# microsoft/Tokenizer

Measured on AMD Instinct MI355X. Metric: input MB/s encoded (cl100k_base), higher is better.
Workload: dtype u8

## Files before the change

tokenizer_amd/csrc/tkz_kernels.hip:

```cpp
#include "tkz_kernels.h"

#include <type_traits>

#include "tkz_bpe.h"
#include "tkz_classes.h"
#include "tkz_corpus.h"
#include "tkz_pretok.h"
#include "tkz_simt.h"

namespace tkz {

TKZ_KERNEL(256) void k_docmark(const int64_t* offs, int64_t n_items, int64_t total, uint64_t* bits, int32_t* counters) {
    const int64_t stride = simt::nblocks() * simt::nthreads();
    for (int64_t d = simt::bid() * simt::nthreads() + simt::tid(); d <= n_items; d += stride) {
        const int64_t pos = offs[d];
        bool ok = pos >= 0 && pos <= total;
        if (d == 0) ok = ok && pos == 0;
        if (d == n_items) ok = ok && pos == total;
        else ok = ok && pos <= offs[d + 1];
        if (!ok) { simt::atomic_or((unsigned*)&counters[0], (unsigned)kErrOffsets); continue; }
        const int64_t w = pos >> 6;
        if (d > 0) { const int64_t prev = offs[d - 1]; if (prev >= 0 && prev <= pos && (prev >> 6) == w) continue; }
        uint64_t m = 1ull << (pos & 63);
        int64_t cur = pos;
// ... 463 lines not shown
    const int w = (s >> 2) + i;
    const uint32_t x = simt::alignbit(s_bytes[w + 1], s_bytes[w], (uint32_t)(s & 3) * 8u);
    const int nb = len - 4 * i;
    return nb >= 4 ? x : (nb <= 0 ? 0u : (x & ((1u << (8 * nb)) - 1u)));
}

constexpr int kProbeLdsBytes = (kSub + kHalo) + 2 * (kSub + 2) + 2 * kMidMax + 4 * kMidMax + 4 * (kSub / 32);
constexpr int kProbeLdsQuads = (kProbeLdsBytes + 15) / 16;
struct ProbeLds { uint32_t* bytes; uint16_t* pstart; uint16_t* mid; uint32_t* midres; uint32_t* mark; const uint4* kmask; };
TKZ_DEV ProbeLds tkz_probe_lds(uint4* wave_quads, const uint4* kmask) {
    ProbeLds L;
    uint8_t* b = reinterpret_cast<uint8_t*>(wave_quads);
    L.bytes = reinterpret_cast<uint32_t*>(b); b += kSub + kHalo;
    L.midres = reinterpret_cast<uint32_t*>(b); b += 4 * kMidMax;
    L.mark = reinterpret_cast<uint32_t*>(b); b += 4 * (kSub / 32);
    L.pstart = reinterpret_cast<uint16_t*>(b); b += 2 * (kSub + 2);
    L.mid = reinterpret_cast<uint16_t*>(b);
    L.kmask = kmask;
    return L;
}
TKZ_DEV void tkz_probe_kmask_init(uint4* s_kmask) {
    if (simt::tid() <= TKZ_SHORT_KEY_MAX) {
        const int len = simt::tid();
        uint32_t m[3];
        for (int i = 0; i < 3; ++i) { const int nb = len - 4 * i; m[i] = nb >= 4 ? 0xFFFFFFFFu : (nb <= 0 ? 0u : ((1u << (8 * nb)) - 1u)); }
        uint4 v; v.x = m[0]; v.y = m[1]; v.z = m[2]; v.w = 0;
        s_kmask[len] = v;
    }
}
struct ProbeText { uint4 v0, v1; };
static_assert((kSub + kHalo) / 16 <= 128, "two 16-byte loads per lane cover the sub-tile and its halo");
TKZ_DEV void tkz_probe_request_text(const EncodeParams& P, int64_t sub, ProbeText* tx) {
    const int lane = simt::lane();
    const int64_t base = sub * kSub;
    uint4 v0, v1;
    v0.x = v0.y = v0.z = v0.w = 0; v1 = v0;
    const int64_t p0 = base + 16 * (int64_t)lane, p1 = base + 16 * (int64_t)(lane + 64);
    if (p0 + 16 <= P.total) v0 = tkz_load16_nt(P.bytes + p0);
    else {
        uint32_t w[4] = {0, 0, 0, 0};
        for (int j = 0; j < 16; ++j) if (p0 + j < P.total) w[j >> 2] |= (uint32_t)P.bytes[p0 + j] << (8 * (j & 3));
        v0.x = w[0]; v0.y = w[1]; v0.z = w[2]; v0.w = w[3];
    }
    if (lane + 64 < (kSub + kHalo) / 16) {
        if (p1 + 16 <= P.total) v1 = tkz_load16_nt(P.bytes + p1);
        else {
            uint32_t w[4] = {0, 0, 0, 0};
            for (int j = 0; j < 16; ++j) if (p1 + j < P.total) w[j >> 2] |= (uint32_t)P.bytes[p1 + j] << (8 * (j & 3));
            v1.x = w[0]; v1.y = w[1]; v1.z = w[2]; v1.w = w[3];
        }
    }
    tx->v0 = v0; tx->v1 = v1;
}
template <bool REPORT>
TKZ_DEV void tkz_probe_subtile(const TkzTables& T, const EncodeParams& P, int64_t sub, const ProbeLds& LD, ProbeText& tx, int64_t next) {
    const int lane = simt::lane();
    uint32_t* s_bytes = LD.bytes;
    uint16_t* s_pstart = LD.pstart;
    uint16_t* s_mid = LD.mid;
    uint32_t* s_midres = LD.midres;
    uint32_t* s_mark = LD.mark;
    const uint4* s_kmask = LD.kmask;
    const uint8_t* sb = reinterpret_cast<const uint8_t*>(s_bytes);
    const int64_t base = sub * kSub;
    const int nb = (int)(P.total - base < kSub ? P.total - base : kSub);
    const uint8_t* gbase = P.bytes + base;
    const bool prof = TKZ_DEV_FLAG(P, 16);
    long long t_0 = prof ? simt::clock() : 0, t_1 = 0, t_2 = 0, t_3 = 0;
    uint4 v0 = tx.v0, v1 = tx.v1;
    uint64_t myword = 0, mymark = 0;
    if (lane < kSub / 64) {
        const int64_t w = sub * (kSub / 64) + lane;
        if (w < P.nwords) { myword = P.startbits[w]; mymark = P.docbits[w]; }
    }
    const int64_t from = base + nb, w0 = from >> 6;
    uint64_t ahead = (w0 + lane < P.nwords) ? P.startbits[w0 + lane] : 0ull;
    const int64_t pb = P.pbase[sub];
    { uint4* s4 = reinterpret_cast<uint4*>(s_bytes); s4[lane] = v0; if (lane + 64 < (kSub + kHalo) / 16) s4[lane + 64] = v1; }
    if (next >= 0) tkz_probe_request_text(P, next, &tx);
    if (lane < kSub / 64) {
        const int lim = nb - lane * 64;
        if (lim <= 0) myword = 0; else if (lim < 64) myword &= tkz_lowmask(lim);
        s_mark[2 * lane] = (uint32_t)mymark; s_mark[2 * lane + 1] = (uint32_t)(mymark >> 32);
    }
    int64_t last_end;
    {
        int64_t found = -1;
        for (int64_t c = 0; found < 0; ++c) {
            const int64_t w = w0 + c * 64 + lane;
            uint64_t v = c == 0 ? ahead : (w < P.nwords ? P.startbits[w] : 0);
            if (w == w0) v &= ~tkz_lowmask((int)(from & 63));
            const uint64_t any = simt::ballot(v != 0);
            if (any) {
                const int src = tkz_ctz64(any);
                const uint32_t lo = simt::shflu((uint32_t)v, src), hi = simt::shflu((uint32_t)(v >> 32), src);
                found = ((w0 + c * 64 + src) << 6) + tkz_ctz64(((uint64_t)hi << 32) | lo);
            } else if (w0 + (c + 1) * 64 >= P.nwords) found = P.total;
        }
        last_end = found;
    }
    const int last_end_rel = (int)(last_end - base < 2 * kSub + 2 ? last_end - base : 2 * kSub + 2);
    const uint32_t wlo = simt::shflu((uint32_t)myword, lane >> 2), whi = simt::shflu((uint32_t)(myword >> 32), lane >> 2);
    const uint32_t bits16 = (uint32_t)(((((uint64_t)whi << 32) | wlo) >> (16 * (lane & 3))) & 0xFFFFull);
    int np;
    {
        int off = tkz_wave_scan<5>(tkz_popc32(bits16), &np);
        for (uint32_t b = bits16; b; b &= b - 1) s_pstart[off++] = (uint16_t)(16 * lane + tkz_ctz32(b));
        if (lane == 0) s_pstart[np] = (uint16_t)last_end_rel;
    }
    (void)simt::ballot(true);
    if (prof) t_1 = simt::clock();
    const char* tb0 = reinterpret_cast<const char*>(T.short_slots);
    const uint32_t mid_off = (uint32_t)(reinterpret_cast<const char*>(T.mid_slots) - tb0);
    int nmid = 0;
#pragma unroll 1
    for (int k0 = 0; k0 < np; k0 += 64) {
        const int k = k0 + lane;
        int len = 0;
        if (k < np) len = (int)s_pstart[k + 1] - (int)s_pstart[k];
        const uint64_t midm = simt::ballot(len > TKZ_SHORT_KEY_MAX && len <= kArenaPiece);
        if ((midm >> lane) & 1ull) s_mid[nmid + tkz_popc64(midm & tkz_lowmask(lane))] = (uint16_t)k;
        nmid += tkz_popc64(midm);
    }
    (void)simt::ballot(true);
#pragma unroll 1
    for (int m0 = 0; m0 < nmid; m0 += 64) {
        const bool valid = m0 + lane < nmid;
        int s = 0, len = 13;
        uint32_t kk[7] = {0, 0, 0, 0, 0, 0, 0}, oa = 0, ob = 0;
        if (valid) {
            const int k = s_mid[m0 + lane];
            s = s_pstart[k];
            len = (int)s_pstart[k + 1] - s;
        }
        const bool is_mid = valid && len <= TKZ_MID_KEY_MAX;
        if (is_mid) {
#pragma unroll
            for (int i = 0; i < 7; ++i) kk[i] = tkz_key_dword(s_bytes, s, len, i);
            uint32_t s1, s2;
            tkz_mid_slots(T, kk, (uint32_t)len, &s1, &s2);
            oa = mid_off + 32u * s1; ob = mid_off + 32u * s2;
        }
        const uint4 a0 = tkz_load16(tb0 + oa), a1 = tkz_load16(tb0 + oa + 16u), b0 = tkz_load16(tb0 + ob), b1 = tkz_load16(tb0 + ob + 16u);
        int32_t rank = TKZ_RANK_NONE;
        if (is_mid) rank = tkz_match_mid(kk, (uint32_t)len, a0, a1, b0, b1);
        else if (valid) {
            if (s + len <= kSub + kHalo) rank = tkz_lookup_long(T, [&](int i) -> uint32_t { return sb[s + i]; }, (uint32_t)len);
            else rank = tkz_lookup_long(T, [&](int i) -> uint32_t { return gbase[s + i]; }, (uint32_t)len);
        }
        if (valid) s_midres[m0 + lane] = (uint32_t)rank;
    }
    (void)simt::ballot(true);
    if (prof) t_2 = simt::clock();
    uint32_t* const ml = P.mlist + sub * (int64_t)P.mcap;
    uint4* const mq = P.mquad + sub * (int64_t)P.mcap;
    int ns = 0, nl = 0, midseen = 0;
    int promo_extra = 0;
    bool giant = false, coopl = false;
    constexpr int U = TKZ_PROBE_U;
#ifdef TKZ_DEVPROF
    long long pf_first = 0, pf_second = 0, pf_emit = 0, pf_t = 0;
    int pf_batches = 0, pf_valid = 0, pf_want2 = 0, pf_iters2 = 0;
#define TKZ_PROBE_MARK(acc) do { if (prof) { const long long pf_now = simt::clock(); acc += pf_now - pf_t; pf_t = pf_now; } } while (0)
    if (prof) pf_t = simt::clock();
#else
#define TKZ_PROBE_MARK(acc) do { } while (0)
#endif
#pragma unroll 1
    for (int k0 = 0; k0 < np; k0 += 64 * U) {
        int ps[U], plen[U];
        uint32_t hs[U], kw0[U], kw1[U], kw2[U];
        uint4 a0[U], a1[U];
#pragma unroll
        for (int u = 0; u < U; ++u) {
            const int k = k0 + 64 * u + lane;
            ps[u] = 0; plen[u] = 0;
            if (k < np) { ps[u] = s_pstart[k]; plen[u] = (int)s_pstart[k + 1] - ps[u]; }
            const int s = ps[u], w = s >> 2;
            const uint32_t sh = (uint32_t)(s & 3) * 8u;
            const uint32_t d0 = s_bytes[w], d1 = s_bytes[w + 1], d2 = s_bytes[w + 2], d3 = s_bytes[w + 3];
            const bool is_short = plen[u] >= 1 && plen[u] <= TKZ_SHORT_KEY_MAX;
            const uint4 km = s_kmask[is_short ? plen[u] : 0];
            kw0[u] = simt::alignbit(d1, d0, sh) & km.x; kw1[u] = simt::alignbit(d2, d1, sh) & km.y; kw2[u] = simt::alignbit(d3, d2, sh) & km.z;
            const uint32_t slot = tkz_short_slot_first(T, kw0[u], kw1[u], kw2[u], (uint32_t)plen[u], &hs[u]);
            const uint32_t oa = is_short ? 16u * slot : 0u;
            a0[u] = tkz_load16(tb0 + oa); a1[u] = tkz_load16(tb0 + oa + 16u);
        }
        int32_t rk[U];
        bool more = false;
#pragma unroll
        for (int u = 0; u < U; ++u) {
            const bool is_short = plen[u] >= 1 && plen[u] <= TKZ_SHORT_KEY_MAX;
            rk[u] = tkz_match_short2x(kw0[u], kw1[u], kw2[u], (uint32_t)plen[u], a0[u], a1[u]);
            more = more || (is_short && rk[u] == TKZ_RANK_NONE);
        }
        bool two_pass = simt::ballot(more) != 0;
        TKZ_PROBE_MARK(pf_first);
#ifdef TKZ_DEVPROF
        if (prof) {
            for (int u = 0; u < U; ++u) { const int nv = np - (k0 + 64 * u); if (nv > 0) { ++pf_batches; pf_valid += nv < 64 ? nv : 64; } }
            for (int u = 0; u < U; ++u) pf_want2 += tkz_popc64(simt::ballot(plen[u] >= 1 && plen[u] <= TKZ_SHORT_KEY_MAX && rk[u] == TKZ_RANK_NONE));
            pf_iters2 += two_pass ? 1 : 0;
            pf_t = simt::clock();
        }
#endif
        if (two_pass) {
#pragma unroll
            for (int u = 0; u < U; ++u) {
                const bool want = plen[u] >= 1 && plen[u] <= TKZ_SHORT_KEY_MAX && rk[u] == TKZ_RANK_NONE;
                if (want) {
                    const uint32_t ob = 16u * tkz_short_slot_second(T, hs[u]);
                    a0[u] = tkz_load16(tb0 + ob); a1[u] = tkz_load16(tb0 + ob + 16u);
                }
            }
#pragma unroll
            for (int u = 0; u < U; ++u) {
                const bool want = plen[u] >= 1 && plen[u] <= TKZ_SHORT_KEY_MAX && rk[u] == TKZ_RANK_NONE;
                if (want) rk[u] = tkz_match_short2x(kw0[u], kw1[u], kw2[u], (uint32_t)plen[u], a0[u], a1[u]);
            }
        }
        TKZ_PROBE_MARK(pf_second);
#pragma unroll
        for (int u = 0; u < U; ++u) {
            const int k = k0 + 64 * u + lane;
            const bool valid = k < np;
            const int s = ps[u], len = plen[u];
            const bool is_mid = len > TKZ_SHORT_KEY_MAX && len <= kArenaPiece;
            const uint64_t midm = simt::ballot(is_mid);
            int32_t rank = rk[u];
            if (is_mid) rank = (int32_t)s_midres[midseen + tkz_popc64(midm & tkz_lowmask(lane))];
            midseen += tkz_popc64(midm);
            const bool is_giant = len > kArenaPiece;
            const bool miss = valid && !is_giant && rank == TKZ_RANK_NONE;
            if (P.pextra) {
                const uint32_t ex = (valid && !is_giant && !miss && ((uint32_t)rank & kPromoFlag)) ? (((uint32_t)rank >> kPromoCntShift) & 3u) : 0u;
                promo_extra += (int)ex;
            }
            const bool miss_s = miss && len <= kShortMax, miss_l = miss && len > kShortMax;
            const uint64_t sm = simt::ballot(miss_s), lm = simt::ballot(miss_l);
            const int is_ = ns + tkz_popc64(sm & tkz_lowmask(lane)), il = nl + tkz_popc64(lm & tkz_lowmask(lane));
            ns += tkz_popc64(sm); nl += tkz_popc64(lm);
            const uint32_t ent = (uint32_t)s | ((uint32_t)(len - 1) << kMrLenShift);
            if (miss_s && is_ + nl < P.mcap) {
                ml[is_] = ent;
                uint4 kq; kq.x = kw0[u]; kq.y = kw1[u]; kq.z = kw2[u]; kq.w = 0;
                if (len > TKZ_SHORT_KEY_MAX) { kq.x = tkz_key_dword(s_bytes, s, len, 0); kq.y = tkz_key_dword(s_bytes, s, len, 1); kq.z = tkz_key_dword(s_bytes, s, len, 2); kq.w = tkz_key_dword(s_bytes, s, len, 3); }
                mq[is_] = kq;
            }
            if (miss_l && il + ns < P.mcap) ml[P.mcap - 1 - il] = ent;
            uint32_t rec = ((s_mark[s >> 5] >> (s & 31)) & 1u) ? kPrMark : 0u;
            if (REPORT) giant = giant || (miss_l && len > kSmallLanePiece);
            else coopl = coopl || (miss_l && len > P.lane_piece);
            if (is_giant) { rec |= kPrMiss | kPrGiant | (uint32_t)s; giant = giant || valid; }
            else if (miss) rec |= kPrMiss | (miss_l ? (kPrLong | (uint32_t)il) : (uint32_t)is_);
            else rec |= (uint32_t)rank;
            if (valid && pb + k < P.prank_cap) tkz_store_nt(&P.prank[pb + k], (int32_t)rec);
        }
        TKZ_PROBE_MARK(pf_emit);
    }
#undef TKZ_PROBE_MARK
#ifdef TKZ_DEVPROF
    if (prof && lane == 0) {
        simt::atomic_add64(&P.devprof[48], (unsigned long long)pf_first); simt::atomic_add64(&P.devprof[49], (unsigned long long)pf_second);
        simt::atomic_add64(&P.devprof[50], (unsigned long long)pf_emit); simt::atomic_add64(&P.devprof[51], (unsigned long long)pf_batches);
        simt::atomic_add64(&P.devprof[52], (unsigned long long)pf_valid); simt::atomic_add64(&P.devprof[53], (unsigned long long)pf_want2);
        simt::atomic_add64(&P.devprof[54], (unsigned long long)pf_iters2);
    }
#endif
    if (prof && lane == 0) {
        t_3 = simt::clock();
        simt::atomic_add64(&P.devprof[0], 1); simt::atomic_add64(&P.devprof[1], (unsigned long long)(t_3 - t_0));
        simt::atomic_add64(&P.devprof[2], (unsigned long long)(t_1 - t_0)); simt::atomic_add64(&P.devprof[3], (unsigned long long)(t_3 - t_2));
        simt::atomic_add64(&P.devprof[4], (unsigned long long)(t_2 - t_1)); simt::atomic_add64(&P.devprof[5], (unsigned long long)nmid);
        simt::atomic_add64(&P.devprof[6], (unsigned long long)np);
    }
    const uint32_t f = (nl ? 1u : 0u) | (simt::ballot(giant) ? 2u : 0u) | (simt::ballot(coopl) ? 4u : 0u);
    if (P.pextra) { int tot; (void)tkz_wave_scan_sum(promo_extra, &tot); promo_extra = tot; }
    if (lane == 0) {
        P.heavy_flag[sub] = (uint8_t)f;
        P.mcount[sub] = (uint32_t)ns | ((uint32_t)nl << 16);
        if (P.pextra) P.pextra[sub] = promo_extra;
        if (!REPORT && P.tc_atomic) P.tile_count[sub] = 0;
        if (REPORT && ns + nl > P.mcap) { simt::atomic_or((unsigned*)&P.counters[0], (unsigned)kErrMissCap); simt::atomic_max((unsigned*)&P.counters[1], (unsigned)(ns + nl)); }
        if (pb + np > P.prank_cap) simt::atomic_or((unsigned*)&P.counters[0], (unsigned)kErrCapacity);
    }
}
TKZ_KERNEL_OCC(256, TKZ_PROBE_OCC) void k_probe(TkzTables T, EncodeParams P) {
    TKZ_SHARED uint4 s_wave[kThreads / 64][kProbeLdsQuads];
    TKZ_SHARED uint4 s_kmask[TKZ_SHORT_KEY_MAX + 1];
    tkz_probe_kmask_init(s_kmask);
    simt::sync();
    const int64_t sub0 = (tkz_xcd_block(simt::bid(), simt::nblocks()) * (kThreads / 64) + simt::wave()) * kProbePer;
    if (sub0 >= P.nsub) return;
    const ProbeLds LD = tkz_probe_lds(s_wave[simt::wave()], s_kmask);
    ProbeText tx;
    tkz_probe_request_text(P, sub0, &tx);
#pragma unroll 1
    for (int it = 0; it < kProbePer && sub0 + it < P.nsub; ++it) {
        const int64_t nxt = (it + 1 < kProbePer && sub0 + it + 1 < P.nsub) ? sub0 + it + 1 : -1;
        tkz_probe_subtile<false>(T, P, sub0 + it, LD, tx, nxt);
        (void)simt::ballot(true);
    }
}

struct alignas(4) TkzDwords4 { uint32_t x, y, z, w; };
TKZ_DEV void tkz_load_piece16(const uint8_t* bytes, int64_t total, int64_t abs, uint32_t* pw) {
    const int64_t a0 = abs & ~(int64_t)3;
    const uint32_t sh = (uint32_t)(abs & 3) * 8u;
    uint32_t w[5];
    if (a0 + 20 <= total) {
        const TkzDwords4 v = *reinterpret_cast<const TkzDwords4*>(bytes + a0);
        w[0] = v.x; w[1] = v.y; w[2] = v.z; w[3] = v.w;
        w[4] = *reinterpret_cast<const uint32_t*>(bytes + a0 + 16);
    } else {
#pragma unroll
        for (int i = 0; i < 5; ++i) {
            const int64_t p = a0 + 4 * i;
            if (p + 4 <= total) w[i] = *reinterpret_cast<const uint32_t*>(bytes + p);
            else { w[i] = 0; for (int j = 0; j < 4; ++j) if (p + j < total) w[i] |= (uint32_t)bytes[p + j] << (8 * j); }
        }
    }
#pragma unroll
    for (int i = 0; i < 4; ++i) pw[i] = simt::alignbit(w[i + 1], w[i], sh);
}

TKZ_HD uint32_t tkz_result_entry(bool dense, int cnt, int off) { return kMrDone | (dense ? kMrDense : 0u) | ((uint32_t)(cnt - 1) << kMrCntShift) | (uint32_t)off; }
TKZ_HD uint32_t tkz_result_inline(int cnt) { return kMrDone | kMrInline | ((uint32_t)(cnt - 1) << kMrCntShift); }
TKZ_HD int tkz_result_cnt(uint32_t r) { return (int)((r >> kMrCntShift) & 1023u) + 1; }
TKZ_HD int tkz_result_off(uint32_t r) { return (int)(r & kMrOffMask); }

template <int N, class Pre>
TKZ_DEV int tkz_find_list(const Pre* pre, int g) {
    int q = 0;
#pragma unroll
    for (int step = N / 2; step >= 1; step >>= 1) if (pre[q + step] <= g) q += step;
    return q;
}

constexpr int kMsStride = TkzBpeGeom<16>::kStride, kMsIdStride = TkzBpeGeom<16>::kIdStride;
#ifndef TKZ_MS_SHORT_LEN
#define TKZ_MS_SHORT_LEN 8
#endif
#ifndef TKZ_MS_TWO_MIN
#define TKZ_MS_TWO_MIN 320
#endif
constexpr int kMsTwoListsMin = TKZ_MS_TWO_MIN;
constexpr int kMsShortLen = TKZ_MS_SHORT_LEN;
struct MsLds { uint4* pr; uint32_t* ids; uint16_t* rec; uint16_t* idx; int* extra; uint16_t* pre; const uint16_t* brank16; };
constexpr int kMsLdsBytes = kMsStride * 64 * 4 + kMsIdStride * 64 * 4 + 2 * (2 * 64 + 2 * 64) + 4 * kGroup + 2 * (kGroup + 1);
constexpr int kMsLdsQuads = (kMsLdsBytes + 15) / 16;
static_assert((kMsThreads / 64) * kMsLdsQuads * 16 + 512 <= 40960, "k_merge_short: four workgroups a CU (160 KB of LDS, allocated in units of 1,280 bytes)");
TKZ_DEV MsLds tkz_ms_lds(uint4* wave_quads, const uint16_t* brank16) {
    MsLds L;
    uint8_t* b = reinterpret_cast<uint8_t*>(wave_quads);
    L.pr = reinterpret_cast<uint4*>(b); b += kMsStride * 64 * 4;
    L.ids = reinterpret_cast<uint32_t*>(b); b += kMsIdStride * 64 * 4;
    L.extra = reinterpret_cast<int*>(b); b += 4 * kGroup;
    L.rec = reinterpret_cast<uint16_t*>(b); b += 2 * 2 * 64;
    L.idx = reinterpret_cast<uint16_t*>(b); b += 2 * 2 * 64;
    L.pre = reinterpret_cast<uint16_t*>(b);
    L.brank16 = brank16;
    return L;
}
TKZ_DEV void tkz_ms_brank_init(const TkzTables& T, uint16_t* s_brank16) {
    for (int i = simt::tid(); i < 256; i += simt::nthreads()) {
        const uint32_t v = (uint32_t)T.byte_rank[i];
        s_brank16[i] = (uint16_t)(v >= (uint32_t)TKZ_PSEUDO_BASE ? 0xFFFFu : (v < 0xFFFEu ? v : 0xFFFEu));
    }
}
TKZ_DEV void tkz_merge_short_group(const TkzTables& T, const EncodeParams& P, int64_t grp, const MsLds& LD) {
    constexpr int NMAX = 16, STRIDE = kMsStride, IDSTRIDE = kMsIdStride;
    static_assert(kGroup == 16 && kShortMax == 16, "list entries: 4 bits of sub-tile, 10 of index; 10 of relpos, 4 of length, 1 flag");
    const int lane = simt::lane();
    const uint16_t* s_brank16 = LD.brank16;
    auto byte_id = [&](uint32_t b) -> uint32_t {
        const uint32_t v = s_brank16[b];
        return v < 0xFFFEu ? v : (v == 0xFFFFu ? (uint32_t)TKZ_PSEUDO_BASE + b : (uint32_t)T.byte_rank[b]);
    };
    auto pair_rank = [&](uint32_t b0, uint32_t b1) -> int32_t { return T.bytepair_rank[(b0 << 8) | b1]; };
    const int64_t sub0 = grp * kGroup;
    if (sub0 >= P.nsub) return;
    uint16_t* s_rec = LD.rec;
    uint16_t* s_idx = LD.idx;
    int* s_extra = LD.extra;
    uint16_t* s_pre = LD.pre;
    uint32_t* ids = LD.ids + lane * IDSTRIDE;
    uint32_t* pr = reinterpret_cast<uint32_t*>(LD.pr) + lane * STRIDE;
    int my_np = 0, my_ns = 0;
    if (lane < kGroup && sub0 + lane < P.nsub) { my_np = P.pcount[sub0 + lane]; my_ns = (int)(P.mcount[sub0 + lane] & 0xFFFFu); }
    { const int nl_ = lane < kGroup && sub0 + lane < P.nsub ? (int)(P.mcount[sub0 + lane] >> 16) : 0; if (my_ns + nl_ > P.mcap) my_ns = 0; }
    int ntotal;
    { const int pre = tkz_wave_scan_sum(my_ns, &ntotal); if (lane <= kGroup) s_pre[lane] = (uint16_t)pre; }
    if (lane < kGroup) s_extra[lane] = 0;
    uint32_t* const ml0 = P.mlist + sub0 * (int64_t)P.mcap;
    int err = 0, dused = 0, done = 0;
    int nl0 = 0, nl1 = 0;
    int st_look = 0, st_hit = 0;
    int32_t* const dense = P.dense + grp * kDenseCap;
    const bool memo = T.memo_n != 0;
    const bool sparse = T.memo_hits_sparse != 0;
    const bool count_hits = T.memo_hits != nullptr && (!sparse || (grp & 7) == 0);
    auto assign = [&](bool have, int cnt, int si, int j, int rel) -> int32_t* {
        int btot;
        const bool big = have && cnt > 4;
        const int doff = dused + tkz_wave_scan_sum(big ? cnt : 0, &btot);
        int32_t* dst = nullptr;
        if (have) {
            if (!big) ml0[si * (int64_t)P.mcap + j] = tkz_result_inline(cnt);
            else {
                const bool packed = doff + cnt <= kDenseCap;
                dst = packed ? dense + doff : P.tmp + ((sub0 + si) * kSub + rel);
                ml0[si * (int64_t)P.mcap + j] = tkz_result_entry(packed, cnt, packed ? doff : rel);
            }
            if (cnt > 1) simt::atomic_add(&s_extra[si], cnt - 1);
        }
        dused += btot;
        return dst;
    };
    uint4* const mq0 = P.mquad + sub0 * (int64_t)P.mcap;
    auto key_of = [&](uint4 kq, int len, uint32_t* kw, bool* nul) {
        kw[0] = kq.x; kw[1] = kq.y; kw[2] = kq.z; kw[3] = kq.w;
        uint32_t z = 0;
#pragma unroll
        for (int i = 0; i < 4; ++i) {
            const int nb = len - 4 * i;
            const uint32_t m = nb >= 4 ? 0xFFFFFFFFu : (nb <= 0 ? 0u : ((1u << (8 * nb)) - 1u));
            z |= (kw[i] - 0x01010101u) & ~kw[i] & 0x80808080u & m;
        }
        *nul = z != 0;
    };
    auto memo_phase = [&](int take, uint32_t r16, uint32_t ix, uint4 fkq) -> bool {
        (void)simt::ballot(true);
        const bool mine = lane < take;
        const int si = (int)(ix >> 10), j = (int)(ix & 1023u), rel = (int)(r16 & 1023u), len = (int)((r16 >> 10) & 15u) + 1;
        bool hit = false;
        uint32_t hit_slot = 0;
        uint4 vv; vv.x = vv.y = vv.z = vv.w = 0;
        if (mine && memo) {
            uint32_t kw[4];
            bool nul;
            key_of(fkq, len, kw, &nul);
            const uint32_t b = tkz_mulhi(tkz_hash_memo(kw, (uint32_t)len), T.memo_n / kMemoWays) * kMemoWays;
#pragma unroll
            for (int wy = 0; wy < (int)kMemoWays; ++wy) {
                const TkzMemoSlot* slot = &T.memo[b + wy];
                const uint4 kk = tkz_load16(&slot->k[0]);
                const uint4 v = tkz_load16(&slot->v[0]);
// ... 1895 lines not shown
```

tokenizer_amd/csrc/tkz_simt.h:

```cpp
#pragma once
#include <stdint.h>

#ifdef TKZ_HOSTEMU
#include "hip_emu.h"
#else
#include <hip/hip_runtime.h>

#define TKZ_DEV __device__ __forceinline__
#define TKZ_HD __host__ __device__ __forceinline__
#define TKZ_KERNEL(bounds) __global__ __launch_bounds__(bounds)
#define TKZ_KERNEL_OCC(bounds, waves_per_simd) __global__ __launch_bounds__(bounds, waves_per_simd)
#define TKZ_SHARED __shared__
#define TKZ_LAUNCH(kernel, grid, block, stream, ...) \
    hipLaunchKernelGGL(kernel, dim3((unsigned)(grid)), dim3((unsigned)(block)), 0, (stream), __VA_ARGS__)

namespace simt {
TKZ_DEV int tid() { return (int)threadIdx.x; }
TKZ_DEV int lane() { return (int)(threadIdx.x & 63); }
TKZ_DEV int wave() { return __builtin_amdgcn_readfirstlane((int)(threadIdx.x >> 6)); }
TKZ_DEV uint64_t uniform64(uint64_t v) {
    return ((uint64_t)(uint32_t)__builtin_amdgcn_readfirstlane((int)(uint32_t)(v >> 32)) << 32) | (uint32_t)__builtin_amdgcn_readfirstlane((int)(uint32_t)v);
}
TKZ_DEV int64_t bid() { return (int64_t)blockIdx.x; }
TKZ_DEV int64_t nblocks() { return (int64_t)gridDim.x; }
TKZ_DEV int nthreads() { return (int)blockDim.x; }
TKZ_DEV void sync() { __syncthreads(); }
TKZ_DEV uint64_t ballot(bool p) { return __ballot(p ? 1 : 0); }
TKZ_DEV int shfl(int v, int src) { return __shfl(v, src, 64); }
TKZ_DEV uint32_t shflu(uint32_t v, int src) { return (uint32_t)__shfl((int)v, src, 64); }
TKZ_DEV int shfl_up(int v, int d) { return __shfl_up(v, (unsigned)d, 64); }
TKZ_DEV int shfl_xor(int v, int m) { return __shfl_xor(v, m, 64); }
TKZ_DEV int first_lane(int v) { return __builtin_amdgcn_readfirstlane(v); }
TKZ_DEV int atomic_add(int* p, int v) { return atomicAdd(p, v); }
TKZ_DEV unsigned atomic_or(unsigned* p, unsigned v) { return atomicOr(p, v); }
TKZ_DEV unsigned atomic_and(unsigned* p, unsigned v) { return atomicAnd(p, v); }
TKZ_DEV unsigned atomic_max(unsigned* p, unsigned v) { return atomicMax(p, v); }
TKZ_DEV unsigned atomic_cas(unsigned* p, unsigned expect, unsigned v) { return atomicCAS(p, expect, v); }
TKZ_DEV void fence() { __threadfence(); }
TKZ_DEV unsigned long long atomic_or64(unsigned long long* p, unsigned long long v) { return atomicOr(p, v); }
TKZ_DEV unsigned long long atomic_add64(unsigned long long* p, unsigned long long v) { return atomicAdd(p, v); }
TKZ_DEV unsigned long long atomic_min64(unsigned long long* p, unsigned long long v) { return atomicMin(p, v); }
TKZ_DEV unsigned long long atomic_max64(unsigned long long* p, unsigned long long v) { return atomicMax(p, v); }
TKZ_DEV long long clock() { return (long long)__builtin_readcyclecounter(); }
template <int CTRL> TKZ_DEV int dpp_mov(int v) { return __builtin_amdgcn_mov_dpp(v, CTRL, 0xf, 0xf, false); }
TKZ_DEV int scan_inclusive(int v) {
    const int l = lane();
    int x = v, t;
    t = dpp_mov<0x111>(x); if ((l & 15) >= 1) x += t;
    t = dpp_mov<0x112>(x); if ((l & 15) >= 2) x += t;
    t = dpp_mov<0x114>(x); if ((l & 15) >= 4) x += t;
    t = dpp_mov<0x118>(x); if ((l & 15) >= 8) x += t;
    t = dpp_mov<0x142>(x); if ((l & 31) >= 16) x += t;
    t = dpp_mov<0x143>(x); if (l >= 32) x += t;
    return x;
}
TKZ_DEV int last_lane(int v) { return __builtin_amdgcn_readlane(v, 63); }
TKZ_DEV uint32_t wave_min_u32(uint32_t v) {
    const int l = lane();
    uint32_t x = v, t;
    t = (uint32_t)dpp_mov<0x111>((int)x); if ((l & 15) >= 1) x = t < x ? t : x;
    t = (uint32_t)dpp_mov<0x112>((int)x); if ((l & 15) >= 2) x = t < x ? t : x;
    t = (uint32_t)dpp_mov<0x114>((int)x); if ((l & 15) >= 4) x = t < x ? t : x;
    t = (uint32_t)dpp_mov<0x118>((int)x); if ((l & 15) >= 8) x = t < x ? t : x;
    t = (uint32_t)dpp_mov<0x142>((int)x); if ((l & 31) >= 16) x = t < x ? t : x;
    t = (uint32_t)dpp_mov<0x143>((int)x); if (l >= 32) x = t < x ? t : x;
    return (uint32_t)__builtin_amdgcn_readlane((int)x, 63);
}
TKZ_DEV uint32_t alignbit(uint32_t hi, uint32_t lo, uint32_t sh) { return __builtin_amdgcn_alignbit(hi, lo, sh); }
}
typedef uint32_t tkz_u32x4 __attribute__((ext_vector_type(4)));
TKZ_DEV uint4 tkz_load16_nt(const void* p) {
    const tkz_u32x4 v = __builtin_nontemporal_load(reinterpret_cast<const tkz_u32x4*>(p));
    uint4 r; r.x = v.x; r.y = v.y; r.z = v.z; r.w = v.w; return r;
}
TKZ_DEV uint32_t tkz_load_nt(const uint32_t* p) { return __builtin_nontemporal_load(p); }
TKZ_DEV uint32_t tkz_atomic_load_agent(const uint32_t* p) { return __hip_atomic_load(p, __ATOMIC_RELAXED, __HIP_MEMORY_SCOPE_AGENT); }
TKZ_DEV int32_t tkz_load_nt(const int32_t* p) { return __builtin_nontemporal_load(p); }
TKZ_DEV void tkz_store_nt(int32_t* p, int32_t v) { __builtin_nontemporal_store(v, p); }
TKZ_DEV void tkz_store16_nt(void* p, uint4 v) {
    tkz_u32x4 x; x.x = v.x; x.y = v.y; x.z = v.z; x.w = v.w;
    __builtin_nontemporal_store(x, reinterpret_cast<tkz_u32x4*>(p));
}
#endif

TKZ_HD int tkz_popc64(uint64_t x) { return __builtin_popcountll(x); }
TKZ_HD int tkz_popc32(uint32_t x) { return __builtin_popcount(x); }
#ifdef TKZ_HOSTEMU
#include <cstdio>
#include <cstdlib>
#define TKZ_NONZERO(x, what) do { if (!(x)) { fprintf(stderr, "tkz: %s(0) is undefined\n", what); abort(); } } while (0)
#else
#define TKZ_NONZERO(x, what) ((void)0)
#endif
TKZ_HD int tkz_ctz64(uint64_t x) { TKZ_NONZERO(x, "tkz_ctz64"); return __builtin_ctzll(x); }
TKZ_HD int tkz_ctz32(uint32_t x) { TKZ_NONZERO(x, "tkz_ctz32"); return __builtin_ctz(x); }
TKZ_HD int tkz_msb64(uint64_t x) { TKZ_NONZERO(x, "tkz_msb64"); return 63 - __builtin_clzll(x); }
TKZ_HD int tkz_msb32(uint32_t x) { TKZ_NONZERO(x, "tkz_msb32"); return 31 - __builtin_clz(x); }
TKZ_HD int tkz_ctz64z(uint64_t x) { return x ? __builtin_ctzll(x) : 64; }
TKZ_HD uint64_t tkz_brev64(uint64_t x) {
    x = ((x >> 1) & 0x5555555555555555ull) | ((x & 0x5555555555555555ull) << 1);
    x = ((x >> 2) & 0x3333333333333333ull) | ((x & 0x3333333333333333ull) << 2);
    x = ((x >> 4) & 0x0F0F0F0F0F0F0F0Full) | ((x & 0x0F0F0F0F0F0F0F0Full) << 4);
    return __builtin_bswap64(x);
}
TKZ_HD uint64_t tkz_lowmask(int n) { return n >= 64 ? ~0ull : ((1ull << n) - 1ull); }
```

tokenizer_amd/csrc/tkz_tables.h:

```cpp
#pragma once
#include <stdint.h>

#include "tkz_simt.h"

#define TKZ_RANK_NONE 0x7FFFFFFF
#define TKZ_PSEUDO_BASE 0x7FFFFC00
#define TKZ_MAX_RANK ((1 << 27) - 2)

#define TKZ_SHORT_KEY_MAX 12
#define TKZ_MID_KEY_MAX 28

struct alignas(16) TkzShortSlot {
    uint32_t k0, k1, k2;
    uint32_t rank_len;
};
#define TKZ_SHORT_RANK_BITS 27
#define TKZ_SHORT_RANK_MASK ((1u << TKZ_SHORT_RANK_BITS) - 1u)

struct alignas(16) TkzMidSlot {
    uint32_t k[7];
    uint32_t rank_len;
};

struct alignas(16) TkzLongSlot {
    uint32_t hash;
    int32_t rank;
    uint32_t off;
    uint32_t len;
};

struct alignas(16) TkzPairSlot {
    uint32_t a, b;
    int32_t rank;
    uint32_t valid;
};
#define TKZ_PAIR_CID_LIMIT 0x1FFF00u
TKZ_HD uint32_t tkz_pair_cid(uint32_t id) { return id >= (uint32_t)TKZ_PSEUDO_BASE ? id - (uint32_t)TKZ_PSEUDO_BASE + TKZ_PAIR_CID_LIMIT : id; }
TKZ_HD uint64_t tkz_pair_key42(uint32_t a, uint32_t b) { return (uint64_t)tkz_pair_cid(a) | ((uint64_t)tkz_pair_cid(b) << 21); }

struct alignas(16) TkzMemoSlot { uint32_t k[4]; uint32_t v[4]; };
constexpr uint32_t kMemoValid = 0x80000000u, kMemoBusy = 0xFFFFFFFFu;
#ifndef TKZ_MEMO_WAYS
#define TKZ_MEMO_WAYS 1
#endif
constexpr uint32_t kMemoWays = TKZ_MEMO_WAYS;

constexpr uint32_t kPromoFlag = 1u << 26, kPromoIdxMask = (1u << 22) - 1u;
constexpr int kPromoCntShift = 22;
constexpr uint32_t kPromoMaxEntries = 1u << 22;
constexpr uint32_t kMemoHitsSat = 64;

struct TkzTables {
    TkzMemoSlot* memo; uint32_t memo_n;
    uint32_t* memo_hits; uint32_t memo_hits_sparse;
    const uint4* promo; uint32_t promo_n;
    const TkzShortSlot* short_slots; uint32_t short_nb; uint32_t short_seed;
    const TkzMidSlot* mid_slots;     uint32_t mid_ns;   uint32_t mid_seed;
    const TkzLongSlot* long_slots;   uint32_t long_mask;
    const uint8_t* long_blob;
    const TkzPairSlot* pair_slots;   uint32_t pair_n; uint32_t pair_seed; uint32_t pair_compact;
    const int32_t* byte_rank;
    const int32_t* bytepair_rank;
    const uint8_t* bmp_class;
    int32_t max_key_len;
    int32_t pattern;
    int32_t max_rank;
};

struct TkzDecodeTable {
    const uint32_t* off;
    const uint8_t* blob;
    const int32_t* ids;
    int64_t n;
    int32_t dense;
};

TKZ_HD uint32_t tkz_mix32(uint32_t h) {
    h ^= h >> 16; h *= 0x7feb352dU; h ^= h >> 15; h *= 0x846ca68bU; h ^= h >> 16;
    return h;
}
TKZ_HD uint32_t tkz_rotl(uint32_t x, int r) { return (x << r) | (x >> (32 - r)); }
TKZ_HD uint32_t tkz_fmix(uint32_t h) { h ^= h >> 16; h *= 0x7feb352dU; h ^= h >> 15; return h; }
TKZ_HD uint32_t tkz_mulhi(uint32_t h, uint32_t n) { return (uint32_t)(((uint64_t)h * (uint64_t)n) >> 32); }
TKZ_HD uint32_t tkz_hash_second(uint32_t h1) { const uint32_t h = h1 * 0x846ca68bU + 0x165667B1u; return h ^ (h >> 15); }
TKZ_HD uint32_t tkz_hash_short(uint32_t k0, uint32_t k1, uint32_t k2, uint32_t len, uint32_t seed) {
    uint32_t h = (k0 ^ tkz_rotl(k1, 13) ^ tkz_rotl(k2, 23) ^ (len << 27) ^ seed) * 0x9E3779B1u;
    return tkz_fmix(h ^ (h >> 15) ^ k1);
}
TKZ_HD uint32_t tkz_hash_short2(uint32_t h1) { return tkz_hash_second(h1); }
TKZ_HD uint32_t tkz_hash_memo(const uint32_t* k, uint32_t len) {
    const uint32_t h = (k[0] ^ tkz_rotl(k[1], 13) ^ tkz_rotl(k[2], 23) ^ tkz_rotl(k[3], 7) ^ (len << 27)) * 0x9E3779B1u;
    return tkz_fmix(h ^ (h >> 15) ^ k[1] ^ k[3]);
}
TKZ_HD uint32_t tkz_hash_mid(const uint32_t* k, uint32_t len, uint32_t seed) {
    uint32_t h = (k[0] + seed) * 0x9E3779B1u;
    h ^= tkz_rotl(k[1] * 0x85EBCA77u, 15);
    h ^= tkz_rotl(k[2] * 0xC2B2AE3Du, 7);
    h += tkz_rotl(k[3] * 0x27D4EB2Fu, 11);
    h ^= tkz_rotl(k[4] * 0x165667B1u, 19);
    h += tkz_rotl(k[5] * 0x9E3779B9u, 3);
    h ^= tkz_rotl(k[6] * 0x85EBCA6Bu, 23);
    return tkz_fmix(h + len * 0x27D4EB2Fu);
}
TKZ_HD uint32_t tkz_hash_long_init(uint32_t len) { return 0x2545F491u ^ (len * 0x9E3779B9u); }
TKZ_HD uint32_t tkz_hash_long_step(uint32_t h, uint32_t w) { return tkz_mix32(h ^ w) + 0x632BE5ABu; }
TKZ_HD uint32_t tkz_hash_pair(uint32_t a, uint32_t b, uint32_t seed) {
    return tkz_fmix(((a + seed) * 0x9E3779B1u) ^ tkz_rotl(b * 0x85EBCA77u, 13));
}
TKZ_HD uint32_t tkz_hash_pair2(uint32_t h1) { return tkz_hash_second(h1); }

TKZ_HD uint4 tkz_load16(const void* p) { return *reinterpret_cast<const uint4*>(p); }

TKZ_HD void tkz_short_slots(const TkzTables& T, uint32_t k0, uint32_t k1, uint32_t k2, uint32_t len, uint32_t* s1, uint32_t* s2) {
    const uint32_t h = tkz_hash_short(k0, k1, k2, len, T.short_seed);
    *s1 = 2u * tkz_mulhi(h, T.short_nb); *s2 = 2u * tkz_mulhi(tkz_hash_short2(h), T.short_nb);
}
TKZ_HD uint32_t tkz_short_slot_first(const TkzTables& T, uint32_t k0, uint32_t k1, uint32_t k2, uint32_t len, uint32_t* h) {
    *h = tkz_hash_short(k0, k1, k2, len, T.short_seed);
    return 2u * tkz_mulhi(*h, T.short_nb);
}
TKZ_HD uint32_t tkz_short_slot_second(const TkzTables& T, uint32_t h) { return 2u * tkz_mulhi(tkz_hash_short2(h), T.short_nb); }
TKZ_HD bool tkz_short_slot_is(uint4 v, uint32_t k0, uint32_t k1, uint32_t k2, uint32_t len) {
    return v.x == k0 && v.y == k1 && v.z == k2 && (v.w >> TKZ_SHORT_RANK_BITS) == len;
}
TKZ_HD int32_t tkz_match_short(uint32_t k0, uint32_t k1, uint32_t k2, uint32_t len, uint4 a0, uint4 a1, uint4 b0, uint4 b1) {
    if (tkz_short_slot_is(a0, k0, k1, k2, len)) return (int32_t)(a0.w & TKZ_SHORT_RANK_MASK);
    if (tkz_short_slot_is(a1, k0, k1, k2, len)) return (int32_t)(a1.w & TKZ_SHORT_RANK_MASK);
    if (tkz_short_slot_is(b0, k0, k1, k2, len)) return (int32_t)(b0.w & TKZ_SHORT_RANK_MASK);
    if (tkz_short_slot_is(b1, k0, k1, k2, len)) return (int32_t)(b1.w & TKZ_SHORT_RANK_MASK);
    return TKZ_RANK_NONE;
}
TKZ_HD int32_t tkz_match_short2(uint32_t k0, uint32_t k1, uint32_t k2, uint32_t len, uint4 a0, uint4 a1) {
    if (tkz_short_slot_is(a0, k0, k1, k2, len)) return (int32_t)(a0.w & TKZ_SHORT_RANK_MASK);
    if (tkz_short_slot_is(a1, k0, k1, k2, len)) return (int32_t)(a1.w & TKZ_SHORT_RANK_MASK);
    return TKZ_RANK_NONE;
}
TKZ_HD int32_t tkz_match_short2x(uint32_t k0, uint32_t k1, uint32_t k2, uint32_t len, uint4 a0, uint4 a1) {
    const uint32_t d0 = (a0.x ^ k0) | (a0.y ^ k1) | (a0.z ^ k2) | ((a0.w >> TKZ_SHORT_RANK_BITS) ^ len);
    const uint32_t d1 = (a1.x ^ k0) | (a1.y ^ k1) | (a1.z ^ k2) | ((a1.w >> TKZ_SHORT_RANK_BITS) ^ len);
    const uint32_t r = d0 == 0 ? a0.w : a1.w;
    return ((d0 == 0 || d1 == 0) && len != 0) ? (int32_t)(r & TKZ_SHORT_RANK_MASK) : TKZ_RANK_NONE;
}
TKZ_HD int32_t tkz_lookup_short(const TkzTables& T, uint32_t k0, uint32_t k1, uint32_t k2, uint32_t len) {
    uint32_t s1, s2;
    tkz_short_slots(T, k0, k1, k2, len, &s1, &s2);
    return tkz_match_short(k0, k1, k2, len, tkz_load16(&T.short_slots[s1]), tkz_load16(&T.short_slots[s1 + 1]),
                           tkz_load16(&T.short_slots[s2]), tkz_load16(&T.short_slots[s2 + 1]));
}
TKZ_HD void tkz_mid_slots(const TkzTables& T, const uint32_t* k, uint32_t len, uint32_t* s1, uint32_t* s2) {
    const uint32_t h = tkz_hash_mid(k, len, T.mid_seed);
    *s1 = tkz_mulhi(h, T.mid_ns); *s2 = tkz_mulhi(tkz_hash_short2(h), T.mid_ns);
}
TKZ_HD bool tkz_mid_slot_is(uint4 lo, uint4 hi, const uint32_t* k, uint32_t len) {
    return lo.x == k[0] && lo.y == k[1] && lo.z == k[2] && lo.w == k[3] && hi.x == k[4] && hi.y == k[5] && hi.z == k[6] &&
           (hi.w >> TKZ_SHORT_RANK_BITS) == len - 12u;
}
TKZ_HD int32_t tkz_match_mid(const uint32_t* k, uint32_t len, uint4 a0, uint4 a1, uint4 b0, uint4 b1) {
    if (tkz_mid_slot_is(a0, a1, k, len)) return (int32_t)(a1.w & TKZ_SHORT_RANK_MASK);
    if (tkz_mid_slot_is(b0, b1, k, len)) return (int32_t)(b1.w & TKZ_SHORT_RANK_MASK);
    return TKZ_RANK_NONE;
}
TKZ_HD int32_t tkz_lookup_mid(const TkzTables& T, const uint32_t* k, uint32_t len) {
    uint32_t s1, s2;
    tkz_mid_slots(T, k, len, &s1, &s2);
    const uint4* m = reinterpret_cast<const uint4*>(T.mid_slots);
    return tkz_match_mid(k, len, tkz_load16(&m[2 * s1]), tkz_load16(&m[2 * s1 + 1]), tkz_load16(&m[2 * s2]), tkz_load16(&m[2 * s2 + 1]));
}

TKZ_HD void tkz_pair_slots(const TkzTables& T, uint32_t a, uint32_t b, uint32_t* s1, uint32_t* s2) {
    const uint32_t h = tkz_hash_pair(a, b, T.pair_seed);
    *s1 = tkz_mulhi(h, T.pair_n); *s2 = tkz_mulhi(tkz_hash_pair2(h), T.pair_n);
}
TKZ_HD uint4 tkz_load_pair_slot(const TkzTables& T, uint32_t slot) {
    return *reinterpret_cast<const uint4*>(reinterpret_cast<const char*>(T.pair_slots) + (uint32_t)(slot << 4));
}
TKZ_HD int32_t tkz_match_pair(const TkzTables& T, uint32_t a, uint32_t b, uint4 v1, uint4 v2) {
    if (T.pair_compact) {
        const uint32_t ca = tkz_pair_cid(a), cb = tkz_pair_cid(b);
        const uint32_t wlo = ca | (cb << 21), whi = (cb >> 11) | 0x80000000u, mhi = 0x800003FFu;
        const uint32_t d0 = (v1.x ^ wlo) | ((v1.y & mhi) ^ whi), d1 = (v1.z ^ wlo) | ((v1.w & mhi) ^ whi);
        const uint32_t d2 = (v2.x ^ wlo) | ((v2.y & mhi) ^ whi), d3 = (v2.z ^ wlo) | ((v2.w & mhi) ^ whi);
        const uint32_t hit = (d0 == 0 ? v1.y : 0u) | (d1 == 0 ? v1.w : 0u) | (d2 == 0 ? v2.y : 0u) | (d3 == 0 ? v2.w : 0u);
        return hit ? (int32_t)((hit >> 10) & 0x1FFFFFu) : TKZ_RANK_NONE;
    }
    if (v1.w != 0 && v1.x == a && v1.y == b) return (int32_t)v1.z;
    if (v2.w != 0 && v2.x == a && v2.y == b) return (int32_t)v2.z;
    return TKZ_RANK_NONE;
}
TKZ_HD int32_t tkz_lookup_pair(const TkzTables& T, uint32_t a, uint32_t b) {
    uint32_t s1, s2;
    tkz_pair_slots(T, a, b, &s1, &s2);
    return tkz_match_pair(T, a, b, tkz_load_pair_slot(T, s1), tkz_load_pair_slot(T, s2));
}

template <class ByteAt>
TKZ_HD int32_t tkz_lookup_long(const TkzTables& T, ByteAt at, uint32_t len) {
    if ((int32_t)len > T.max_key_len || len <= TKZ_MID_KEY_MAX) return TKZ_RANK_NONE;
    uint32_t h = tkz_hash_long_init(len);
    for (uint32_t off = 0; off < len; off += 4) {
        uint32_t w = 0;
        for (uint32_t j = 0; j < 4 && off + j < len; ++j) w |= (uint32_t)at(off + j) << (8 * j);
        h = tkz_hash_long_step(h, w);
    }
    uint32_t s = h & T.long_mask;
    for (;;) {
        const uint4 v = tkz_load16(&T.long_slots[s]);
        if (v.w == 0) return TKZ_RANK_NONE;
        if (v.x == h && v.w == len) {
            const uint8_t* k = T.long_blob + v.z;
            uint32_t i = 0;
            while (i < len && k[i] == at(i)) ++i;
            if (i == len) return (int32_t)v.y;
        }
        s = (s + 1) & T.long_mask;
    }
}

template <class ByteAt>
TKZ_HD int32_t tkz_lookup_any(const TkzTables& T, ByteAt at, uint32_t len) {
    if (len == 0) return TKZ_RANK_NONE;
    if (len <= TKZ_MID_KEY_MAX) {
        uint32_t k[7] = {0, 0, 0, 0, 0, 0, 0};
        for (uint32_t i = 0; i < len; ++i) k[i >> 2] |= (uint32_t)at(i) << (8 * (i & 3));
        return len <= TKZ_SHORT_KEY_MAX ? tkz_lookup_short(T, k[0], k[1], k[2], len) : tkz_lookup_mid(T, k, len);
    }
    return tkz_lookup_long(T, at, len);
}
```

Before: 253,900.

## Use buffer loads, wave-mask bookkeeping and mbcnt in short-probe emit loop

Rewrites the short-key probe and emit loop to track per-batch predicates as 64-bit wave masks, using inverse ballot and mbcnt instead of per-lane popcount prefix sums. Hash-table slot loads now go through a raw buffer resource descriptor with 32-bit offsets, and output stores use byte-offset pointers. The capacity check is hoisted under a wave-uniform overflow test. The aim is to cut scalar/vector instruction count, 64-bit address arithmetic and VGPR pressure in the hot probe loop. The len!=0 guard in match_short2x is removed, and its correctness now relies on the masks or hash layout; the bucket indexing changes from slot*16 to bucket*32, which assumes a bucketed table layout.

```diff
diff --git a/tokenizer_amd/csrc/tkz_kernels.hip b/tokenizer_amd/csrc/tkz_kernels.hip
--- a/tokenizer_amd/csrc/tkz_kernels.hip
+++ b/tokenizer_amd/csrc/tkz_kernels.hip
@@ -639,11 +639,15 @@
     }
     (void)simt::ballot(true);
     if (prof) t_2 = simt::clock();
-    uint32_t* const ml = P.mlist + sub * (int64_t)P.mcap;
-    uint4* const mq = P.mquad + sub * (int64_t)P.mcap;
+    const tkz_rsrc tbr = tkz_make_rsrc(T.short_slots);
+    char* const mlb = reinterpret_cast<char*>(P.mlist + sub * (int64_t)P.mcap);
+    char* const mqb = reinterpret_cast<char*>(P.mquad + sub * (int64_t)P.mcap);
+    char* const prb = reinterpret_cast<char*>(P.prank + pb);
+    const int nrec = P.prank_cap - pb >= np ? np : (P.prank_cap - pb > 0 ? (int)(P.prank_cap - pb) : 0);
+    const uint32_t vseed = simt::opaque(T.short_seed);
     int ns = 0, nl = 0, midseen = 0;
     int promo_extra = 0;
-    bool giant = false, coopl = false;
+    uint64_t giantm = 0, cooplm = 0;
     constexpr int U = TKZ_PROBE_U;
 #ifdef TKZ_DEVPROF
     long long pf_first = 0, pf_second = 0, pf_emit = 0, pf_t = 0;
@@ -658,10 +662,12 @@
         int ps[U], plen[U];
         uint32_t hs[U], kw0[U], kw1[U], kw2[U];
         uint4 a0[U], a1[U];
+        uint64_t validm[U];
 #pragma unroll
         for (int u = 0; u < U; ++u) {
             const int k = k0 + 64 * u + lane;
             ps[u] = 0; plen[u] = 0;
+            validm[u] = simt::ballot_mask(k < np);
             if (k < np) { ps[u] = s_pstart[k]; plen[u] = (int)s_pstart[k + 1] - ps[u]; }
             const int s = ps[u], w = s >> 2;
             const uint32_t sh = (uint32_t)(s & 3) * 8u;
@@ -669,24 +675,25 @@
             const bool is_short = plen[u] >= 1 && plen[u] <= TKZ_SHORT_KEY_MAX;
             const uint4 km = s_kmask[is_short ? plen[u] : 0];
             kw0[u] = simt::alignbit(d1, d0, sh) & km.x; kw1[u] = simt::alignbit(d2, d1, sh) & km.y; kw2[u] = simt::alignbit(d3, d2, sh) & km.z;
-            const uint32_t slot = tkz_short_slot_first(T, kw0[u], kw1[u], kw2[u], (uint32_t)plen[u], &hs[u]);
-            const uint32_t oa = is_short ? 16u * slot : 0u;
-            a0[u] = tkz_load16(tb0 + oa); a1[u] = tkz_load16(tb0 + oa + 16u);
+            hs[u] = tkz_hash_short(kw0[u], kw1[u], kw2[u], (uint32_t)plen[u], vseed);
+            const uint32_t bucket = simt::opaque(tkz_mulhi(hs[u], T.short_nb));
+            const uint32_t oa = is_short ? 32u * bucket : 0u;
+            a0[u] = tkz_rsrc_load16(tbr, oa); a1[u] = tkz_rsrc_load16(tbr, oa + 16u);
         }
         int32_t rk[U];
-        bool more = false;
+        bool want[U], more = false;
 #pragma unroll
         for (int u = 0; u < U; ++u) {
-            const bool is_short = plen[u] >= 1 && plen[u] <= TKZ_SHORT_KEY_MAX;
             rk[u] = tkz_match_short2x(kw0[u], kw1[u], kw2[u], (uint32_t)plen[u], a0[u], a1[u]);
-            more = more || (is_short && rk[u] == TKZ_RANK_NONE);
-        }
-        bool two_pass = simt::ballot(more) != 0;
+            want[u] = (uint32_t)(plen[u] - 1) < (uint32_t)TKZ_SHORT_KEY_MAX && rk[u] == TKZ_RANK_NONE;
+            more = more || want[u];
+        }
+        bool two_pass = simt::ballot_mask(more) != 0;
         TKZ_PROBE_MARK(pf_first);
 #ifdef TKZ_DEVPROF
         if (prof) {
             for (int u = 0; u < U; ++u) { const int nv = np - (k0 + 64 * u); if (nv > 0) { ++pf_batches; pf_valid += nv < 64 ? nv : 64; } }
-            for (int u = 0; u < U; ++u) pf_want2 += tkz_popc64(simt::ballot(plen[u] >= 1 && plen[u] <= TKZ_SHORT_KEY_MAX && rk[u] == TKZ_RANK_NONE));
+            for (int u = 0; u < U; ++u) pf_want2 += tkz_popc64(simt::ballot(want[u]));
             pf_iters2 += two_pass ? 1 : 0;
             pf_t = simt::clock();
         }
@@ -694,54 +701,59 @@
         if (two_pass) {
 #pragma unroll
             for (int u = 0; u < U; ++u) {
-                const bool want = plen[u] >= 1 && plen[u] <= TKZ_SHORT_KEY_MAX && rk[u] == TKZ_RANK_NONE;
-                if (want) {
-                    const uint32_t ob = 16u * tkz_short_slot_second(T, hs[u]);
-                    a0[u] = tkz_load16(tb0 + ob); a1[u] = tkz_load16(tb0 + ob + 16u);
+                if (want[u]) {
+                    const uint32_t ob = 32u * simt::opaque(tkz_mulhi(tkz_hash_short2(hs[u]), T.short_nb));
+                    a0[u] = tkz_rsrc_load16(tbr, ob); a1[u] = tkz_rsrc_load16(tbr, ob + 16u);
                 }
             }
 #pragma unroll
             for (int u = 0; u < U; ++u) {
-                const bool want = plen[u] >= 1 && plen[u] <= TKZ_SHORT_KEY_MAX && rk[u] == TKZ_RANK_NONE;
-                if (want) rk[u] = tkz_match_short2x(kw0[u], kw1[u], kw2[u], (uint32_t)plen[u], a0[u], a1[u]);
+                if (want[u]) rk[u] = tkz_match_short2x(kw0[u], kw1[u], kw2[u], (uint32_t)plen[u], a0[u], a1[u]);
             }
         }
         TKZ_PROBE_MARK(pf_second);
 #pragma unroll
         for (int u = 0; u < U; ++u) {
             const int k = k0 + 64 * u + lane;
-            const bool valid = k < np;
+            const bool valid = simt::lanes(validm[u]);
             const int s = ps[u], len = plen[u];
             const bool is_mid = len > TKZ_SHORT_KEY_MAX && len <= kArenaPiece;
-            const uint64_t midm = simt::ballot(is_mid);
+            const uint64_t midm = simt::ballot_mask(is_mid);
             int32_t rank = rk[u];
-            if (is_mid) rank = (int32_t)s_midres[midseen + tkz_popc64(midm & tkz_lowmask(lane))];
+            if (is_mid) rank = (int32_t)s_midres[simt::mbcnt(midm, midseen)];
             midseen += tkz_popc64(midm);
-            const bool is_giant = len > kArenaPiece;
-            const bool miss = valid && !is_giant && rank == TKZ_RANK_NONE;
+            const uint64_t gm = simt::ballot_mask(len > kArenaPiece);
+            const uint64_t missm = validm[u] & ~gm & simt::ballot_mask(rank == TKZ_RANK_NONE);
+            const uint64_t longm = simt::ballot_mask(len > kShortMax);
+            const uint64_t sm = missm & ~longm, lm = missm & longm;
+            const bool is_giant = simt::lanes(gm), miss = simt::lanes(missm), miss_l = simt::lanes(lm);
             if (P.pextra) {
                 const uint32_t ex = (valid && !is_giant && !miss && ((uint32_t)rank & kPromoFlag)) ? (((uint32_t)rank >> kPromoCntShift) & 3u) : 0u;
                 promo_extra += (int)ex;
             }
-            const bool miss_s = miss && len <= kShortMax, miss_l = miss && len > kShortMax;
-            const uint64_t sm = simt::ballot(miss_s), lm = simt::ballot(miss_l);
-            const int is_ = ns + tkz_popc64(sm & tkz_lowmask(lane)), il = nl + tkz_popc64(lm & tkz_lowmask(lane));
+            const int is_ = simt::mbcnt(sm, ns), il = simt::mbcnt(lm, nl);
             ns += tkz_popc64(sm); nl += tkz_popc64(lm);
+            uint64_t puts = sm, putl = lm;
+            if (ns + nl > P.mcap) {
+                __asm__ volatile("");
+                puts &= simt::ballot_mask(is_ + nl < P.mcap); putl &= simt::ballot_mask(il + ns < P.mcap);
+            }
             const uint32_t ent = (uint32_t)s | ((uint32_t)(len - 1) << kMrLenShift);
-            if (miss_s && is_ + nl < P.mcap) {
-                ml[is_] = ent;
+            if (simt::lanes(puts)) {
+                *reinterpret_cast<uint32_t*>(mlb + 4u * (uint32_t)is_) = ent;
                 uint4 kq; kq.x = kw0[u]; kq.y = kw1[u]; kq.z = kw2[u]; kq.w = 0;
                 if (len > TKZ_SHORT_KEY_MAX) { kq.x = tkz_key_dword(s_bytes, s, len, 0); kq.y = tkz_key_dword(s_bytes, s, len, 1); kq.z = tkz_key_dword(s_bytes, s, len, 2); kq.w = tkz_key_dword(s_bytes, s, len, 3); }
-                mq[is_] = kq;
-            }
-            if (miss_l && il + ns < P.mcap) ml[P.mcap - 1 - il] = ent;
-            uint32_t rec = ((s_mark[s >> 5] >> (s & 31)) & 1u) ? kPrMark : 0u;
-            if (REPORT) giant = giant || (miss_l && len > kSmallLanePiece);
-            else coopl = coopl || (miss_l && len > P.lane_piece);
-            if (is_giant) { rec |= kPrMiss | kPrGiant | (uint32_t)s; giant = giant || valid; }
+                *reinterpret_cast<uint4*>(mqb + 16u * (uint32_t)is_) = kq;
+            }
+            if (simt::lanes(putl)) *reinterpret_cast<uint32_t*>(mlb + 4u * (uint32_t)(P.mcap - 1 - il)) = ent;
+            uint32_t rec = ((s_mark[s >> 5] >> (s & 31)) & 1u) << 30;
+            if (REPORT) giantm |= lm & simt::ballot_mask(len > kSmallLanePiece);
+            else cooplm |= lm & simt::ballot_mask(len > P.lane_piece);
+            giantm |= gm;
+            if (is_giant) rec |= kPrMiss | kPrGiant | (uint32_t)s;
             else if (miss) rec |= kPrMiss | (miss_l ? (kPrLong | (uint32_t)il) : (uint32_t)is_);
             else rec |= (uint32_t)rank;
-            if (valid && pb + k < P.prank_cap) tkz_store_nt(&P.prank[pb + k], (int32_t)rec);
+            if (k < nrec) tkz_store_nt(reinterpret_cast<int32_t*>(prb + simt::opaque(4u * (uint32_t)k)), (int32_t)rec);
         }
         TKZ_PROBE_MARK(pf_emit);
     }
@@ -761,7 +773,7 @@
         simt::atomic_add64(&P.devprof[4], (unsigned long long)(t_2 - t_1)); simt::atomic_add64(&P.devprof[5], (unsigned long long)nmid);
         simt::atomic_add64(&P.devprof[6], (unsigned long long)np);
     }
-    const uint32_t f = (nl ? 1u : 0u) | (simt::ballot(giant) ? 2u : 0u) | (simt::ballot(coopl) ? 4u : 0u);
+    const uint32_t f = (nl ? 1u : 0u) | (giantm ? 2u : 0u) | (cooplm ? 4u : 0u);
     if (P.pextra) { int tot; (void)tkz_wave_scan_sum(promo_extra, &tot); promo_extra = tot; }
     if (lane == 0) {
         P.heavy_flag[sub] = (uint8_t)f;
@@ -779,7 +791,7 @@
     simt::sync();
     const int64_t sub0 = (tkz_xcd_block(simt::bid(), simt::nblocks()) * (kThreads / 64) + simt::wave()) * kProbePer;
     if (sub0 >= P.nsub) return;
-    const ProbeLds LD = tkz_probe_lds(s_wave[simt::wave()], s_kmask);
+    const ProbeLds LD = tkz_probe_lds(s_wave[simt::tid() >> 6], s_kmask);
     ProbeText tx;
     tkz_probe_request_text(P, sub0, &tx);
 #pragma unroll 1
diff --git a/tokenizer_amd/csrc/tkz_simt.h b/tokenizer_amd/csrc/tkz_simt.h
--- a/tokenizer_amd/csrc/tkz_simt.h
+++ b/tokenizer_amd/csrc/tkz_simt.h
@@ -67,6 +67,17 @@
     return (uint32_t)__builtin_amdgcn_readlane((int)x, 63);
 }
 TKZ_DEV uint32_t alignbit(uint32_t hi, uint32_t lo, uint32_t sh) { return __builtin_amdgcn_alignbit(hi, lo, sh); }
+TKZ_DEV uint64_t ballot_mask(bool p) { return __builtin_amdgcn_ballot_w64(p); }
+TKZ_DEV bool lanes(uint64_t m) { return __builtin_amdgcn_inverse_ballot_w64(m); }
+TKZ_DEV int mbcnt(uint64_t m, int base = 0) { return (int)__builtin_amdgcn_mbcnt_hi((uint32_t)(m >> 32), __builtin_amdgcn_mbcnt_lo((uint32_t)m, (uint32_t)base)); }
+TKZ_DEV uint32_t opaque(uint32_t v) { __asm__("" : "+v"(v)); return v; }
+}
+typedef __amdgpu_buffer_rsrc_t tkz_rsrc;
+TKZ_DEV tkz_rsrc tkz_make_rsrc(const void* base) { return __builtin_amdgcn_make_buffer_rsrc(const_cast<void*>(base), (short)0, 0x7FFFFFFF, 0x00020000); }
+TKZ_DEV uint4 tkz_rsrc_load16(tkz_rsrc r, uint32_t off) {
+    typedef uint32_t u32x4 __attribute__((ext_vector_type(4)));
+    const u32x4 v = __builtin_amdgcn_raw_buffer_load_b128(r, off, 0, 0);
+    uint4 x; x.x = v.x; x.y = v.y; x.z = v.z; x.w = v.w; return x;
 }
 typedef uint32_t tkz_u32x4 __attribute__((ext_vector_type(4)));
 TKZ_DEV uint4 tkz_load16_nt(const void* p) {
@@ -104,3 +115,15 @@
     return __builtin_bswap64(x);
 }
 TKZ_HD uint64_t tkz_lowmask(int n) { return n >= 64 ? ~0ull : ((1ull << n) - 1ull); }
+
+#ifdef TKZ_HOSTEMU
+namespace simt {
+inline uint64_t ballot_mask(bool p) { return ballot(p); }
+inline bool lanes(uint64_t m) { return (m >> lane()) & 1ull; }
+inline int mbcnt(uint64_t m, int base = 0) { return base + tkz_popc64(m & tkz_lowmask(lane())); }
+inline uint32_t opaque(uint32_t v) { return v; }
+}
+typedef const char* tkz_rsrc;
+inline tkz_rsrc tkz_make_rsrc(const void* base) { return reinterpret_cast<const char*>(base); }
+inline uint4 tkz_rsrc_load16(tkz_rsrc r, uint32_t off) { return *reinterpret_cast<const uint4*>(r + off); }
+#endif
diff --git a/tokenizer_amd/csrc/tkz_tables.h b/tokenizer_amd/csrc/tkz_tables.h
--- a/tokenizer_amd/csrc/tkz_tables.h
+++ b/tokenizer_amd/csrc/tkz_tables.h
@@ -139,7 +139,7 @@
     const uint32_t d0 = (a0.x ^ k0) | (a0.y ^ k1) | (a0.z ^ k2) | ((a0.w >> TKZ_SHORT_RANK_BITS) ^ len);
     const uint32_t d1 = (a1.x ^ k0) | (a1.y ^ k1) | (a1.z ^ k2) | ((a1.w >> TKZ_SHORT_RANK_BITS) ^ len);
     const uint32_t r = d0 == 0 ? a0.w : a1.w;
-    return ((d0 == 0 || d1 == 0) && len != 0) ? (int32_t)(r & TKZ_SHORT_RANK_MASK) : TKZ_RANK_NONE;
+    return (d0 == 0 || d1 == 0) ? (int32_t)(r & TKZ_SHORT_RANK_MASK) : TKZ_RANK_NONE;
 }
 TKZ_HD int32_t tkz_lookup_short(const TkzTables& T, uint32_t k0, uint32_t k1, uint32_t k2, uint32_t len) {
     uint32_t s1, s2;
```

Result: faster. 257,400, median of 6 (+1.4%).
